# ai-forever/Kandinsky-2

Hardware: NVIDIA H100
Metric: unet_denoising_steps_per_sec (higher is better)
Workload: dtype f16

## Files before the change

kandinsky-2_b200/csrc/k2_api.cu:

```cuda
#include <stdio.h>
#include <stdlib.h>
#include <string.h>

#include <algorithm>
#include <atomic>
#include <mutex>

#include "../../include/k2b200.h"
#include "k2_internal.h"

namespace k2 {

static thread_local std::string g_err;
static std::atomic<long long> g_launches{0};
static int g_force_bn = 0;
static int g_force_split = 0;
static int g_pdl = 0;


void set_error(const std::string& msg) { g_err = msg; }
int fail(const std::string& msg) {
  g_err = msg;
  return -1;
}
// ... 316 lines not shown
                        static_cast<uint64_t>(NB)};
    uint64_t str[3] = {static_cast<uint64_t>(src.ld) * 2, static_cast<uint64_t>(src.ld) * 2 * W,
                       static_cast<uint64_t>(src.ld) * 2 * W * H};
    uint32_t box[4] = {64, static_cast<uint32_t>(p.TW), static_cast<uint32_t>(p.TH), static_cast<uint32_t>(p.TN)};
    if (encode_tmap_f16(&p.tmA[s], src.ptr, 4, dims, str, box)) return -1;
  }
  const int BN = pl.BN, splits = pl.splits, fuse_stats = pl.fuse_stats;
  p.splits = splits;
  p.k_per_split = (kchunks + splits - 1) / splits;
  p.M_total = static_cast<long long>(NB) * H * W * (up2 ? 4 : 1);
  p.ws = reinterpret_cast<float*>(workspace);
  p.n_tiles = (Cout + BN - 1) / BN;
  p.Cout = Cout;
  {
    uint64_t dims[3] = {static_cast<uint64_t>(Ktot), static_cast<uint64_t>(w_rows), static_cast<uint64_t>(w_batched ? NB : 1)};
    uint64_t str[2] = {static_cast<uint64_t>(ldw) * 2,
                       (w_batched ? static_cast<uint64_t>(w_batch_stride) : static_cast<uint64_t>(ldw) * w_rows) * 2};
    uint32_t box[3] = {64, static_cast<uint32_t>(BN), 1};
    if (encode_tmap_f16(&p.tmB, w_packed, 3, dims, str, box)) return -1;
  }
  p.bias = bias;
  p.residual = reinterpret_cast<const __half*>(residual);
  p.ldr = ldr;
  p.out = out;
  p.ldo = ldo;
  p.out_mode = (splits > 1) ? 2 : out_mode;
  p.gn_part = (fuse_stats == 1) ? reinterpret_cast<float2*>(gn_partial) : nullptr;
  p.gn_mode = (fuse_stats == 1) ? (p.TN == 1 ? 1 : 2) : 0;
  if (out_mode == 0) {
    K2_REQUIRE(ldo % 8 == 0 && (reinterpret_cast<uintptr_t>(out) & 15) == 0, "conv_gemm: out alignment");
    if (residual)
      K2_REQUIRE(ldr % 8 == 0 && (reinterpret_cast<uintptr_t>(residual) & 15) == 0, "conv_gemm: residual alignment");
  }
  int rc = launch_conv_gemm(p, BN, pl.es, static_cast<cudaStream_t>(stream));
  if (rc == 0) g_launches.fetch_add(1, std::memory_order_relaxed);
  if (rc == 0 && splits > 1) {
    rc = launch_splitk_finalize(p.ws, splits, p.M_total, Cout, bias, p.residual, ldr, reinterpret_cast<__half*>(out), ldo,
                                fuse_stats == 2 ? reinterpret_cast<float2*>(gn_partial) : nullptr,
                                static_cast<cudaStream_t>(stream));
    if (rc == 0) g_launches.fetch_add(1, std::memory_order_relaxed);
  }
  return rc;
}

int k2_conv_plan(int NB, int H, int W, int taps, int Ktot, int Cout, int out_mode, long long workspace_bytes,
                 int want_gn_partial, int* info) {
  K2_REQUIRE(NB > 0 && H > 0 && W > 0 && Cout > 0 && info, "conv_plan: bad arguments");
  K2_REQUIRE(Ktot > 0 && Ktot % 64 == 0, "conv_plan: Ktot must be a positive multiple of 64");
  ConvPlan pl;
  plan_conv(NB, H, W, taps == 9, Ktot / 64, Cout, out_mode, workspace_bytes > 0, workspace_bytes, want_gn_partial != 0, pl);
  plan_to_info(pl, info);
  return 0;
}

}
```

kandinsky-2_b200/csrc/k2_common.cuh:

```cuda
#pragma once
#include <cuda.h>
#include <cuda_fp16.h>
#include <cuda_runtime.h>
#include <stdint.h>
#include <stdio.h>

namespace k2 {

__device__ __forceinline__ uint32_t smem_u32(const void* p) {
  return static_cast<uint32_t>(__cvta_generic_to_shared(p));
}

__device__ __forceinline__ uint32_t lane_id() { return threadIdx.x & 31; }

__device__ __forceinline__ bool elect_one() {
  uint32_t pred = 0;
  asm volatile(
      "{\n"
      ".reg .b32 rx;\n"
      ".reg .pred px;\n"
      "elect.sync rx|px, 0xffffffff;\n"
      "selp.b32 %0, 1, 0, px;\n"
      "}\n"
      : "=r"(pred));
// ... 51 lines not shown
  asm volatile("fence.proxy.async.shared::cta;" ::: "memory");
}

__device__ __forceinline__ void tma_prefetch_desc(const CUtensorMap* tm) {
  asm volatile("prefetch.tensormap [%0];" ::"l"(reinterpret_cast<uint64_t>(tm)) : "memory");
}
__device__ __forceinline__ void tma_load_2d(void* dst, const CUtensorMap* tm, uint64_t* bar, int c0,
                                            int c1) {
  asm volatile(
      "cp.async.bulk.tensor.2d.shared::cluster.global.mbarrier::complete_tx::bytes [%0], [%1, {%3, "
      "%4}], [%2];"
      ::"r"(smem_u32(dst)),
      "l"(reinterpret_cast<uint64_t>(tm)), "r"(smem_u32(bar)), "r"(c0), "r"(c1)
      : "memory");
}
__device__ __forceinline__ void tma_load_3d(void* dst, const CUtensorMap* tm, uint64_t* bar, int c0,
                                            int c1, int c2) {
  asm volatile(
      "cp.async.bulk.tensor.3d.shared::cluster.global.mbarrier::complete_tx::bytes [%0], [%1, {%3, "
      "%4, %5}], [%2];"
      ::"r"(smem_u32(dst)),
      "l"(reinterpret_cast<uint64_t>(tm)), "r"(smem_u32(bar)), "r"(c0), "r"(c1), "r"(c2)
      : "memory");
}
__device__ __forceinline__ void tma_load_4d(void* dst, const CUtensorMap* tm, uint64_t* bar, int c0,
                                            int c1, int c2, int c3) {
  asm volatile(
      "cp.async.bulk.tensor.4d.shared::cluster.global.mbarrier::complete_tx::bytes [%0], [%1, {%3, "
      "%4, %5, %6}], [%2];"
      ::"r"(smem_u32(dst)),
      "l"(reinterpret_cast<uint64_t>(tm)), "r"(smem_u32(bar)), "r"(c0), "r"(c1), "r"(c2), "r"(c3)
      : "memory");
}

__device__ __forceinline__ uint64_t make_wgmma_desc(uint32_t smem_addr) {
  uint64_t d = 0;
  d |= static_cast<uint64_t>((smem_addr & 0x3FFFF) >> 4);
  d |= static_cast<uint64_t>(1) << 16;
  d |= static_cast<uint64_t>(1024 >> 4) << 32;
  d |= static_cast<uint64_t>(1) << 62;
  return d;
}
__device__ __forceinline__ void wgmma_fence() { asm volatile("wgmma.fence.sync.aligned;" ::: "memory"); }
__device__ __forceinline__ void wgmma_commit() { asm volatile("wgmma.commit_group.sync.aligned;" ::: "memory"); }
template <int N>
__device__ __forceinline__ void wgmma_wait() {
  asm volatile("wgmma.wait_group.sync.aligned %0;" ::"n"(N) : "memory");
}
__device__ __forceinline__ void wgmma_m64n16k16(float (&d)[8], uint64_t adesc, uint64_t bdesc, uint32_t accumulate) {
  asm volatile(
      "{\n"
      ".reg .pred p;\n"
      "setp.ne.b32 p, %10, 0;\n"
      "wgmma.mma_async.sync.aligned.m64n16k16.f32.f16.f16 "
      "{%0, %1, %2, %3, %4, %5, %6, %7}, %8, %9, p, 1, 1, 0, 0;\n"
      "}\n"
      : "+f"(d[0]), "+f"(d[1]), "+f"(d[2]), "+f"(d[3]), "+f"(d[4]), "+f"(d[5]), "+f"(d[6]), "+f"(d[7])
      : "l"(adesc), "l"(bdesc), "r"(accumulate));
}

__device__ __forceinline__ void wgmma_m64n64k16(float (&d)[32], uint64_t adesc, uint64_t bdesc, uint32_t accumulate) {
  asm volatile(
      "{\n"
      ".reg .pred p;\n"
      "setp.ne.b32 p, %34, 0;\n"
      "wgmma.mma_async.sync.aligned.m64n64k16.f32.f16.f16 "
// ... 99 lines not shown
  asm volatile(
      "mma.sync.aligned.m16n8k16.row.col.f32.f16.f16.f32 {%0, %1, %2, %3}, {%4, %5, %6, %7}, {%8, %9}, "
      "{%0, %1, %2, %3};"
      : "+f"(d[0]), "+f"(d[1]), "+f"(d[2]), "+f"(d[3])
      : "r"(a[0]), "r"(a[1]), "r"(a[2]), "r"(a[3]), "r"(b0), "r"(b1));
}
__device__ __forceinline__ void ldmatrix_x4(uint32_t (&r)[4], uint32_t saddr) {
  asm volatile("ldmatrix.sync.aligned.m8n8.x4.shared.b16 {%0, %1, %2, %3}, [%4];"
               : "=r"(r[0]), "=r"(r[1]), "=r"(r[2]), "=r"(r[3])
               : "r"(saddr));
}
__device__ __forceinline__ void ldmatrix_x4_trans(uint32_t (&r)[4], uint32_t saddr) {
  asm volatile("ldmatrix.sync.aligned.m8n8.x4.trans.shared.b16 {%0, %1, %2, %3}, [%4];"
               : "=r"(r[0]), "=r"(r[1]), "=r"(r[2]), "=r"(r[3])
               : "r"(saddr));
}
__device__ __forceinline__ void cp_async_16(uint32_t saddr, const void* gptr, int src_bytes) {
  asm volatile("cp.async.cg.shared.global [%0], [%1], 16, %2;" ::"r"(saddr), "l"(gptr), "r"(src_bytes) : "memory");
}
__device__ __forceinline__ void cp_async_commit() { asm volatile("cp.async.commit_group;" ::: "memory"); }
template <int N>
__device__ __forceinline__ void cp_async_wait() {
  asm volatile("cp.async.wait_group %0;" ::"n"(N) : "memory");
}

__device__ __forceinline__ void sts_v4(uint32_t saddr, uint32_t a, uint32_t b, uint32_t c, uint32_t d) {
  asm volatile("st.shared.v4.b32 [%0], {%1, %2, %3, %4};" ::"r"(saddr), "r"(a), "r"(b), "r"(c), "r"(d) : "memory");
}
__device__ __forceinline__ uint4 lds_v4(uint32_t saddr) {
  uint4 v;
  asm volatile("ld.shared.v4.b32 {%0, %1, %2, %3}, [%4];" : "=r"(v.x), "=r"(v.y), "=r"(v.z), "=r"(v.w) : "r"(saddr) : "memory");
  return v;
}
__device__ __forceinline__ uint32_t lds_u32(uint32_t saddr) {
  uint32_t v;
  asm volatile("ld.shared.b32 %0, [%1];" : "=r"(v) : "r"(saddr) : "memory");
  return v;
}
__device__ __forceinline__ void named_bar_sync(int id, int count) {
  asm volatile("bar.sync %0, %1;" ::"r"(id), "r"(count) : "memory");
}
__device__ __forceinline__ void named_bar_arrive(int id, int count) {
  asm volatile("bar.arrive %0, %1;" ::"r"(id), "r"(count) : "memory");
}
__device__ __forceinline__ void pdl_wait() { asm volatile("griddepcontrol.wait;" ::: "memory"); }
__device__ __forceinline__ void pdl_launch() { asm volatile("griddepcontrol.launch_dependents;" ::: "memory"); }

__device__ __forceinline__ float silu_f(float x) {
  float e, r;
  asm("ex2.approx.ftz.f32 %0, %1;" : "=f"(e) : "f"(-1.44269504088896341f * x));
  asm("rcp.approx.ftz.f32 %0, %1;" : "=f"(r) : "f"(1.f + e));
  return x * r;
}

}
```

kandinsky-2_b200/csrc/k2_conv_gemm.cu:

```cuda
#include <stdio.h>

#include "k2_common.cuh"
#include "k2_internal.h"

namespace k2 {

namespace {

constexpr int BM = 128;
constexpr int BK = 64;
constexpr int A_STAGE_BYTES = BM * BK * 2;
constexpr int ACC_PAD = 4;

constexpr int EPI_STAGE_FLOATS = 32 * 33;
constexpr int EPI_BYTES = 4 * EPI_STAGE_FLOATS * 4 + 4 * 256 * 4;
constexpr int SMEM_LIMIT = 227 * 1024;

template <int BN, int ES>
struct Cfg {
  static constexpr int B_STAGE_BYTES = BN * BK * 2;
  static constexpr int STAGE_BYTES = A_STAGE_BYTES + B_STAGE_BYTES;
  static constexpr int BNC = (BN < 64) ? BN : (ES == 2 ? 128 : 64);
  static_assert(ES == 1 || BN % 128 == 0, "two epilogue sets need N tiles of 128 or 256");
  static constexpr int ACC_BYTES = BM * (BNC + ACC_PAD) * 4;
  static constexpr int BAR_BYTES = 256;
  static constexpr int FIXED = ACC_BYTES + ES * EPI_BYTES + BAR_BYTES + 1024;
  static constexpr int STAGES = (SMEM_LIMIT - FIXED) / STAGE_BYTES > 6 ? 6 : (SMEM_LIMIT - FIXED) / STAGE_BYTES;
  static constexpr int SMEM_BYTES = STAGES * STAGE_BYTES + FIXED;
  static_assert(STAGES >= 2, "conv_gemm: shared memory does not hold two pipeline stages");
};

__device__ __forceinline__ void decode_m_tile(const ConvGemmParams& p, int m_idx, int& n0, int& y0,
                                              int& x0, int& phase) {
  phase = 0;
  if (p.up2) {
    phase = m_idx / p.m_tiles_phase;
    m_idx -= phase * p.m_tiles_phase;
  }
  int tw_i = m_idx % p.tiles_w;
  int t = m_idx / p.tiles_w;
  int th_i = t % p.tiles_h;
  int tn_i = t / p.tiles_h;
  x0 = tw_i * p.TW;
  y0 = th_i * p.TH;
  n0 = tn_i * p.TN;
}

template <int N>
__device__ __forceinline__ void acc_ld(const float* src, uint32_t (&r)[N]) {
#pragma unroll
  for (int v = 0; v < N / 4; ++v) {
    const float4 t = *reinterpret_cast<const float4*>(src + 4 * v);
    r[4 * v] = __float_as_uint(t.x);
    r[4 * v + 1] = __float_as_uint(t.y);
    r[4 * v + 2] = __float_as_uint(t.z);
    r[4 * v + 3] = __float_as_uint(t.w);
  }
}

template <int BN, int ES>
// ... 243 lines not shown
                }
                uint4 ov;
                __half2* oh = reinterpret_cast<__half2*>(&ov);
#pragma unroll
                for (int e = 0; e < 4; ++e) oh[e] = __floats2half2_rn(f[2 * e], f[2 * e + 1]);
                *reinterpret_cast<uint4*>(orow + v * 8) = ov;
              }
            } else {
#pragma unroll
              for (int e = 0; e < CH; ++e) {
                if (col0 + e < p.Cout) {
                  float f = __uint_as_float(r[e]);
                  if (p.bias) f += __ldg(p.bias + col0 + e);
                  if (rrow) f += __half2float(rrow[e]);
                  orow[e] = __float2half_rn(f);
                }
              }
            }
          } else {
            float* o = reinterpret_cast<float*>(p.out);
#pragma unroll
            for (int e = 0; e < CH; ++e) {
              if (col0 + e < p.Cout) {
                float f = __uint_as_float(r[e]);
                if (p.bias) f += __ldg(p.bias + col0 + e);
                o[((static_cast<long long>(n) * p.Cout + (col0 + e)) * p.H + y) * p.W + x] = f;
              }
            }
          }
        }
      }
}


template <int BN, int ES>
__global__ void __launch_bounds__(384, 1) conv_gemm_kernel(const __grid_constant__ ConvGemmParams p) {
  using C = Cfg<BN, ES>;
  constexpr int BNC = C::BNC;
  constexpr int NA = BN / 2;
  extern __shared__ uint8_t smem_raw[];
  uint8_t* smem = reinterpret_cast<uint8_t*>((reinterpret_cast<uintptr_t>(smem_raw) + 1023) &
                                             ~static_cast<uintptr_t>(1023));
  float* acc_smem = reinterpret_cast<float*>(smem + C::STAGES * C::STAGE_BYTES);
  float* stat_smem = reinterpret_cast<float*>(smem + C::STAGES * C::STAGE_BYTES + C::ACC_BYTES);
  uint64_t* full_bar = reinterpret_cast<uint64_t*>(smem + C::STAGES * C::STAGE_BYTES + C::ACC_BYTES + ES * EPI_BYTES);
  uint64_t* empty_bar = full_bar + C::STAGES;

  const int warp_idx = threadIdx.x >> 5;
  const int lane = threadIdx.x & 31;
  const int wg = warp_idx >> 2;

  if (threadIdx.x == 0) {
    tma_prefetch_desc(&p.tmB);
    for (int s = 0; s < 3; ++s)
      if (p.seg_taps[s]) tma_prefetch_desc(&p.tmA[s]);
    for (int i = 0; i < C::STAGES; ++i) {
      mbar_init(&full_bar[i], 1);
      mbar_init(&empty_bar[i], 8);
    }
    fence_barrier_init();
  }
  __syncthreads();
  pdl_wait();
  pdl_launch();

  const int total_tiles = p.m_tiles * p.n_tiles * p.splits;

  if (wg == 0) {
    setmaxnreg_dec<40>();
    if (warp_idx == 0 && elect_one()) {
      int stage = 0;
      uint32_t ring_phase = 0;
      const uint32_t tx_bytes = p.a_box_bytes + C::B_STAGE_BYTES;
      for (int tile = blockIdx.x; tile < total_tiles; tile += gridDim.x) {
        const int n_idx = tile % p.n_tiles;
        const int m_idx = (tile / p.n_tiles) % p.m_tiles;
        const int split = tile / (p.m_tiles * p.n_tiles);
        int n0, y0, x0, phase;
        decode_m_tile(p, m_idx, n0, y0, x0, phase);
        const int kb = phase * p.num_k_chunks;
        const int k0 = split * p.k_per_split;
        const int k1 = min(p.num_k_chunks, k0 + p.k_per_split);
        int s = 0, rem = k0;
        while (rem >= p.seg_taps[s] * p.seg_kchunks[s]) {
          rem -= p.seg_taps[s] * p.seg_kchunks[s];
          ++s;
        }
        int tap = rem / p.seg_kchunks[s];
        int c = rem - tap * p.seg_kchunks[s];
        for (int kc = k0; kc < k1; ++kc) {
          const int taps = p.seg_taps[s];
          const int dy = (taps == 9) ? (tap / 3 - 1) : (taps == 4 ? (tap >> 1) + (phase >> 1) - 1 : 0);
          const int dx = (taps == 9) ? (tap % 3 - 1) : (taps == 4 ? (tap & 1) + (phase & 1) - 1 : 0);
          mbar_wait_lean(&empty_bar[stage], ring_phase ^ 1);
          uint8_t* sA = smem + stage * C::STAGE_BYTES;
          uint8_t* sB = sA + A_STAGE_BYTES;
          mbar_arrive_expect_tx(&full_bar[stage], tx_bytes);
          tma_load_4d(sA, &p.tmA[s], &full_bar[stage], c * BK, x0 + dx, y0 + dy, n0);
          tma_load_3d(sB, &p.tmB, &full_bar[stage], (kb + kc) * BK, n_idx * BN, p.w_batched ? n0 : 0);
          if (++stage == C::STAGES) {
            stage = 0;
            ring_phase ^= 1;
          }
          if (++c == p.seg_kchunks[s]) {
            c = 0;
            if (++tap == taps) {
              tap = 0;
              ++s;
            }
          }
        }
      }
    }
  } else {
    setmaxnreg_inc<232>();
    const int g = wg - 1;
    const int w = warp_idx & 3;
    int stage = 0;
    uint32_t phase = 0;
    for (int tile = blockIdx.x; tile < total_tiles; tile += gridDim.x) {
      const int n_idx = tile % p.n_tiles;
      const int m_idx = (tile / p.n_tiles) % p.m_tiles;
      const int split = tile / (p.m_tiles * p.n_tiles);
      const int nk = min(p.num_k_chunks, (split + 1) * p.k_per_split) - split * p.k_per_split;
      float acc[NA];
#pragma unroll
      for (int i = 0; i < NA; ++i) acc[i] = 0.f;
      int prev_stage = -1;
      for (int kc = 0; kc < nk; ++kc) {
        mbar_wait_lean(&full_bar[stage], phase);
        const uint32_t a_addr = smem_u32(smem + stage * C::STAGE_BYTES) + g * (64 * 128);
        const uint32_t b_addr = smem_u32(smem + stage * C::STAGE_BYTES + A_STAGE_BYTES);
        wgmma_fence();
#pragma unroll
        for (int k = 0; k < BK / 16; ++k) {
          const uint64_t adesc = make_wgmma_desc(a_addr) + static_cast<uint64_t>(k * 2);
          const uint64_t bdesc = make_wgmma_desc(b_addr) + static_cast<uint64_t>(k * 2);
          if constexpr (BN == 256) {
            wgmma_m64n256k16(acc, adesc, bdesc, 1u);
          } else if constexpr (BN == 192) {
            wgmma_m64n192k16(acc, adesc, bdesc, 1u);
          } else if constexpr (BN == 128) {
            wgmma_m64n128k16(acc, adesc, bdesc, 1u);
          } else if constexpr (BN == 64) {
            wgmma_m64n64k16(acc, adesc, bdesc, 1u);
          } else {
            static_assert(BN == 16, "conv_gemm: N tile without a wgmma shape");
            wgmma_m64n16k16(acc, adesc, bdesc, 1u);
          }
        }
        wgmma_commit();
        wgmma_wait<1>();
        if (prev_stage >= 0 && lane == 0) mbar_arrive(&empty_bar[prev_stage]);
        prev_stage = stage;
        if (++stage == C::STAGES) {
          stage = 0;
          phase ^= 1;
        }
      }
      wgmma_wait<0>();
      if (prev_stage >= 0 && lane == 0) mbar_arrive(&empty_bar[prev_stage]);

      int n0, y0, x0, mphase;
      decode_m_tile(p, m_idx, n0, y0, x0, mphase);
      const int r0 = 64 * g + 16 * w + (lane >> 2);
      const int cq = 2 * (lane & 3);
#pragma unroll
      for (int pass = 0; pass < BN / BNC; ++pass) {
        named_bar_sync(3, 256);
#pragma unroll
        for (int i = 0; i < NA; i += 2) {
          if ((8 * (i >> 2)) / BNC != pass) continue;
          const int row = r0 + 8 * ((i >> 1) & 1);
          const int col = 8 * (i >> 2) - pass * BNC + cq;
          *reinterpret_cast<float2*>(acc_smem + row * (BNC + ACC_PAD) + col) = make_float2(acc[i], acc[i + 1]);
        }
        named_bar_sync(3, 256);
        if (ES == 2 || g == 0)
          epilogue_tile<BNC, ES>(p, acc_smem, w, lane, n0, y0, x0, n_idx * BN + pass * BNC, split, m_idx, stat_smem, g,
                                 mphase);
      }
    }
  }
}

__global__ void __launch_bounds__(256) splitk_finalize_kernel(const float* __restrict__ ws, int splits, long long M,
                                                              int Cout, const float* __restrict__ bias,
                                                              const __half* __restrict__ residual, int ldr,
                                                              __half* __restrict__ out, int ldo, float2* __restrict__ gn_part) {
  __shared__ float red[8][32][17];
  const int vx = threadIdx.x & 31, ry = threadIdx.x >> 5;
  const int c0 = (blockIdx.y * 32 + vx) * 8;
  const long long rg = blockIdx.x;
  pdl_wait();
  pdl_launch();
  float st[16];
#pragma unroll
  for (int e = 0; e < 16; ++e) st[e] = 0.f;
  if (c0 < Cout) {
    float bv[8];
#pragma unroll
    for (int e = 0; e < 8; ++e) bv[e] = bias ? __ldg(bias + c0 + e) : 0.f;
#pragma unroll
    for (int rr = 0; rr < 2; ++rr) {
      const long long m = rg * 16 + ry + rr * 8;
      if (m >= M) continue;
      float f[8];
#pragma unroll
      for (int e = 0; e < 8; ++e) f[e] = bv[e];
      for (int s = 0; s < splits; ++s) {
        const float4* w = reinterpret_cast<const float4*>(ws + (static_cast<long long>(s) * M + m) * Cout + c0);
        const float4 a = __ldcs(w), b = __ldcs(w + 1);
        f[0] += a.x; f[1] += a.y; f[2] += a.z; f[3] += a.w; f[4] += b.x; f[5] += b.y; f[6] += b.z; f[7] += b.w;
// ... 10 lines not shown
      }
      uint4 ov;
      __half2* oh = reinterpret_cast<__half2*>(&ov);
#pragma unroll
      for (int e = 0; e < 4; ++e) {
        oh[e] = __floats2half2_rn(f[2 * e], f[2 * e + 1]);
        const float2 t = __half22float2(oh[e]);
        st[2 * e] += t.x;
        st[2 * e + 1] += t.y;
        st[8 + 2 * e] = fmaf(t.x, t.x, st[8 + 2 * e]);
        st[8 + 2 * e + 1] = fmaf(t.y, t.y, st[8 + 2 * e + 1]);
      }
      *reinterpret_cast<uint4*>(out + m * ldo + c0) = ov;
    }
  }
  if (gn_part == nullptr) return;
#pragma unroll
  for (int e = 0; e < 16; ++e) red[ry][vx][e] = st[e];
  __syncthreads();
  const int vx2 = threadIdx.x >> 3, e2 = threadIdx.x & 7;
  const int c = (blockIdx.y * 32 + vx2) * 8 + e2;
  if (c < Cout) {
    float s1 = 0.f, s2 = 0.f;
#pragma unroll
    for (int q = 0; q < 8; ++q) {
      s1 += red[q][vx2][e2];
      s2 += red[q][vx2][8 + e2];
    }
    gn_part[rg * Cout + c] = make_float2(s1, s2);
  }
}


template <int BN, int ES>
int launch_bn(const ConvGemmParams& p, cudaStream_t stream) {
  using C = Cfg<BN, ES>;
  static bool attr_set = false;
  if (!attr_set) {
    K2_CHECK_CUDA(cudaFuncSetAttribute(conv_gemm_kernel<BN, ES>, cudaFuncAttributeMaxDynamicSharedMemorySize,
                                       C::SMEM_BYTES));
    attr_set = true;
  }
  int total = p.m_tiles * p.n_tiles * p.splits;
  int grid = total < num_sms() ? total : num_sms();
  K2_CHECK_CUDA(launch_k(conv_gemm_kernel<BN, ES>, dim3(grid), dim3(384), C::SMEM_BYTES, stream, p));
  return 0;
}

}

int launch_splitk_finalize(const float* ws, int splits, long long M, int Cout, const float* bias, const __half* residual,
                           int ldr, __half* out, int ldo, float2* gn_part, cudaStream_t stream) {
  dim3 grid(static_cast<unsigned int>((M + 15) / 16), (Cout / 8 + 31) / 32);
  K2_CHECK_CUDA(launch_k(splitk_finalize_kernel, grid, dim3(256), 0, stream, ws, splits, M, Cout, bias, residual, ldr, out, ldo,
                         gn_part));
  return 0;
}

int launch_conv_gemm(const ConvGemmParams& p, int BN, int epilogue_sets, cudaStream_t stream) {
  if (epilogue_sets == 2) {
    switch (BN) {
      case 128: return launch_bn<128, 2>(p, stream);
      case 256: return launch_bn<256, 2>(p, stream);
      default: break;
    }
  }
  switch (BN) {
    case 16: return launch_bn<16, 1>(p, stream);
    case 64: return launch_bn<64, 1>(p, stream);
    case 128: return launch_bn<128, 1>(p, stream);
    case 192: return launch_bn<192, 1>(p, stream);
    case 256: return launch_bn<256, 1>(p, stream);
    default: return fail("conv_gemm: unsupported BN");
  }
}

}
```

kandinsky-2_b200/csrc/k2_internal.h:

```cpp
#pragma once
#include <cuda.h>
#include <cuda_fp16.h>
#include <cuda_runtime.h>
#include <stdint.h>

#include <string>

namespace k2 {

void set_error(const std::string& msg);
int fail(const std::string& msg);
#define K2_CHECK_CUDA(expr)                                                                 \
  do {                                                                                      \
    cudaError_t _e = (expr);                                                                \
    if (_e != cudaSuccess)                                                                  \
      return ::k2::fail(std::string(#expr) + ": " + cudaGetErrorString(_e));                \
  } while (0)
#define K2_REQUIRE(cond, msg)                                  \
  do {                                                         \
    if (!(cond)) return ::k2::fail(std::string("k2b200: ") + (msg)); \
  } while (0)

inline bool aligned16(const void* p) { return (reinterpret_cast<uintptr_t>(p) & 15) == 0; }

// ... 17 lines not shown
}
void count_launch(int n = 1);

int encode_tmap_f16(CUtensorMap* out, const void* base, int rank, const uint64_t* dims,
                    const uint64_t* strides_bytes , const uint32_t* box);

struct ConvGemmParams {
  CUtensorMap tmA[3];
  CUtensorMap tmB;
  int w_batched;
  int seg_taps[3];
  int seg_kchunks[3];
  int num_k_chunks;
  int NB, H, W;
  int TN, TH, TW;
  int tiles_n, tiles_h, tiles_w;
  int m_tiles, n_tiles;
  int Cout;
  const float* bias;
  const __half* residual;
  int ldr;
  void* out;
  int ldo;
  int out_mode;
  uint32_t a_box_bytes;
  int splits;
  int k_per_split;
  float* ws;
  long long M_total;
  float2* gn_part;
  int gn_mode;
  int up2;
  int m_tiles_phase;
};
int launch_conv_gemm(const ConvGemmParams& p, int BN, int epilogue_sets, cudaStream_t stream);
int launch_splitk_finalize(const float* ws, int splits, long long M, int Cout, const float* bias, const __half* residual,
                           int ldr, __half* out, int ldo, float2* gn_part, cudaStream_t stream);

struct FlashParams {
  const __half* qkv;
  long long ldq;
  int hs, q_off, k_off, v_off;
  const __half* enc;
  long long lde;
  int ehs, ek_off, ev_off;
  int B, heads, T, Tc;
  __half* out;
  int ldo, ohs;
  float scale_log2e;
};
int gn_apply_blocks_per_sm();
int launch_attention(const FlashParams& p, int head_dim, cudaStream_t stream);

}
```

kandinsky-2_b200/kandinsky2/launch_plan.py:

```python
import gc
import os

import torch

from . import ops

FOLD_MAX_RG = int(os.environ.get("K2_GN_FOLD_MAX_RG", "18"))
TUNE = os.environ.get("K2_AUTOTUNE", "1") != "0"
FORK = os.environ.get("K2_FORK", "1") != "0"
TUNE_SMALL_M = int(os.environ.get("K2_TUNE_SMALL_M", "8192"))
_tune_cache = {}


def tune(key, run, m_rows=0):
    if not TUNE:
        return None
    key = (torch.cuda.current_device(), TUNE_SMALL_M) + key
    if key in _tune_cache:
        return _tune_cache[key]
    info = [0] * 7
    run(None, info)
    bn0, splits = info[0], info[2]
    cout = key[3]
    best = None
    if cout > 64:
        bns = [bn0] if splits > 1 else [bn for bn in (128, 192, 256) if bn - 64 < cout or bn == bn0]
        cands = [(bn0, 0, splits, 1)] + [(bn, 0, splits, es) for bn in bns for es in ((1,) if bn == 192 else (1, 2))
                                        if (bn, es) != (bn0, 1)]
        if 0 < m_rows <= TUNE_SMALL_M and splits == 1:
            for bn in (128, 192, 256):
                if bn - 64 >= cout:
                    continue
                for sp in (2, 3, 4):
                    probe = [0] * 7
                    try:
                        run((bn, 1, sp, 1), probe)
                    except Exception:
                        continue
                    if probe[0] == bn and probe[2] == sp:
                        cands.append((bn, 1, sp, 1))

        def timed(cfg, reps=6):
            run(cfg)
            evs = [torch.cuda.Event(enable_timing=True) for _ in range(reps + 1)]
            evs[0].record()
            for i in range(reps):
                run(cfg)
                evs[i + 1].record()
            torch.cuda.synchronize()
            return min(evs[i].elapsed_time(evs[i + 1]) for i in range(reps))

        t0 = tb = timed(cands[0])
        for cfg in cands[1:]:
            t = timed(cfg)
            if t < tb and t < 0.97 * t0:
                t = max(t, timed(cfg))
                if t < tb and t < 0.97 * t0:
                    best, tb = cfg, t
    _tune_cache[key] = best
    return best
# ... 39 lines not shown
                ev = torch.cuda.Event()
                ev.record()
                self._side_stream.wait_event(ev)
            with torch.cuda.stream(self._side_stream):
                fn()
        self._add(step, kind, flops)

    def _join(self):
        if not self._side_open:
            return
        self._side_open = False

        def step():
            if self._serial:
                return
            ev = torch.cuda.Event()
            ev.record(self._side_stream)
            torch.cuda.current_stream().wait_event(ev)
        self._add(step, "join", 0)

    def _conv(self, srcs, w, cout, out, flops, bias=None, residual=None, want_stats=True, part_slot=None, out_mode=0,
              geom=None, w_batch_stride=0, kind="conv_gemm"):
        part = None
        if want_stats and out_mode == 0:
            g = geom if geom is not None else tuple(out.shape[:3])
            n = ops.gn_part_floats(g[0], g[1], g[2], cout)
            part = self._tmp(part_slot, n, dtype=torch.float32) if part_slot else self._new(n, dtype=torch.float32)
        info = [0] * 7
        run = lambda cfg, info=None: ops.conv_gemm(srcs, w, cout, bias=bias, residual=residual, out=out, gn_part=part,
                                                   info=info, cfg=cfg, out_mode=out_mode, geom=geom,
                                                   w_batch_stride=w_batch_stride)
        key = ("conv", cout, tuple(out.shape), geom, tuple((t.shape[-1], taps) for t, taps in srcs), residual is not None,
               part is not None, out_mode, w_batch_stride > 0)
        cfg = tune(key, run, m_rows=out.shape[0] * out.shape[1] * out.shape[2] if out_mode == 0 and geom is None else 0)
        self._add(lambda: run(cfg, info), kind, flops)
        if part is not None and info[5]:
            self._parts[out.data_ptr()] = (part, info[6] // (geom[0] if geom is not None else out.shape[0]))
        else:
            self._parts.pop(out.data_ptr(), None)

    def _gemm(self, x, w, cout, out, flops, bias=None, residual=None):
        run = lambda cfg, info=None: ops.gemm_rows(x, w, cout, bias=bias, residual=residual, out=out, cfg=cfg, info=info)
        cfg = tune(("gemm", cout, tuple(x.shape), residual is not None), run, m_rows=x.shape[0] * x.shape[1])
        self._add(lambda: run(cfg), "conv_gemm", flops)
        self._parts.pop(out.data_ptr(), None)

    def _stats(self, a, b, eps):
        pa = self._parts.get(a.data_ptr())
        pb = self._parts.get(b.data_ptr()) if b is not None else None
        st = self._new(self.NB, 32, 2, dtype=torch.float32)
        HW = a.shape[1] * a.shape[2]
        if pa is not None and (b is None or pb is not None):
            c1 = b.shape[-1] if b is not None else 0
            self._add(lambda: ops.gn_finalize(pa[0], a.shape[-1], pb[0] if pb else None, c1, self.NB, pa[1], HW, st,
                                              rg1=pb[1] if pb else None, eps=eps), "gn_finalize")
        else:
            self._add(lambda: ops.gn_stats(a, b, stats=st, eps=eps), "gn_stats")
        return st

    def _norm(self, a, b, gamma, beta, y, film=None, act=1, resample=0, xres=None, eps=1e-5):
        pa = self._parts.get(a.data_ptr())
        pb = self._parts.get(b.data_ptr()) if b is not None else None
        have = pa is not None and (b is None or pb is not None)
        cpg = (a.shape[-1] + (b.shape[-1] if b is not None else 0)) // 32
        if have and cpg >= 2 and max(pa[1], pb[1] if pb else 0) <= FOLD_MAX_RG:
            self._add(lambda: ops.gn_apply_fold(a, b, pa[0], pa[1], pb[0] if pb else None, pb[1] if pb else 0, gamma, beta,
                                                film=film, act=act, resample=resample, y=y, xres=xres, eps=eps), "gn_apply")
# ... 66 lines not shown
```

profiles/conv_layers.py:

```python
import argparse
import json
import os
import subprocess
import sys

ROOT = os.path.dirname(os.path.dirname(os.path.abspath(__file__)))
for p in (ROOT, os.path.join(ROOT, "kandinsky-2_b200")):
    if p not in sys.path:
        sys.path.insert(0, p)

import torch

B, H, W = 4, 96, 96


def _card():
    q = subprocess.run(["nvidia-smi", "--query-gpu=name,power.limit,clocks.max.sm", "--format=csv,noheader", "-i", "0"],
                       capture_output=True, text=True)
    return q.stdout.strip() or torch.cuda.get_device_name(0)


def _pad64(c):
    return (c + 63) // 64 * 64

# ... 48 lines not shown
        run(cfg)
    e.record()
    torch.cuda.synchronize()
    reps = max(10, int(min_ms / max(s.elapsed_time(e) / 5, 1e-3)) + 1)
    s.record()
    for _ in range(reps):
        run(cfg)
    e.record()
    torch.cuda.synchronize()
    return s.elapsed_time(e) / reps, reps


def main():
    ap = argparse.ArgumentParser()
    ap.add_argument("--out", default=None)
    ap.add_argument("--min-ms", type=float, default=50.0, help="timed window per configuration")
    ap.add_argument("--mma-n", default="tile", choices=["tile", "64"],
                    help="wgmma N of the build: one instruction per N tile, or m64n64k16 per 64 columns")
    args = ap.parse_args()
    if not torch.cuda.is_available():
        raise SystemExit("needs a CUDA sm_90 device")
    import bench
    from kandinsky2 import launch_plan, ops
    from kandinsky2.model.gaussian_diffusion import FusedStep, create_ddpm_v22
    dev = torch.device("cuda", 0)
    torch.cuda.set_device(dev)
    ops.set_tuning(4, 1)
    res = {"card": _card(), "torch": torch.__version__, "geometry": f"cfg-2: UNet batch {2 * B}, {H}x{W} latents",
           "mma_n": args.mma_n, "min_ms": args.min_ms}

    counts = {}
    tune = launch_plan.tune

    def counting_tune(key, run, m_rows=0):
        counts[key] = counts.get(key, 0) + 1
        return tune(key, run, m_rows=m_rows)
    launch_plan.tune = counting_tune
    model = bench.build_unet(dev)
    image_emb = torch.randn(2 * B, 1280, generator=torch.Generator().manual_seed(1234)).to(dev)
    step = FusedStep(model, B, H, W, dict(image_emb=image_emb), guidance_scale=4.0, cond_first=False, clip_range=2.0,
                     threshold_mode=0)
    launch_plan.tune = tune
    diffusion = create_ddpm_v22(50)
    coef, ts = diffusion._tables(dev)
    order = torch.arange(diffusion.num_timesteps - 1, -1, -1, device=dev)
    step.set_schedule(ts[order], coef[order], torch.randn(len(order), B, 4, H, W, device=dev))
    x = step.latent()
    x.copy_(torch.randn(B, 4, H, W, device=dev))
    step.advance(x)
    torch.cuda.synchronize()
    res["plan_conv_launches"] = sum(1 for _, kind, _ in step.plan.steps if kind == "conv_gemm")
    res["counted_conv_launches"] = sum(counts.values())

    g = torch.Generator(device=dev).manual_seed(7)
    layers = []
    for key, n in counts.items():
        run, shp = _layer(key, dev, g)
        if run is None:
            continue
        info = [0] * 7
        picked = launch_plan._tune_cache.get((dev.index, launch_plan.TUNE_SMALL_M) + key)
        run(picked, info)
        picked_cfg = [info[0], 0, info[2], (picked[3] if picked and picked[3] else 1)]
        cout = shp["N"]
        cfgs = []
        if cout > 64:
            cfgs = [(bn, 0, 1, es) for bn in (128, 192, 256) if bn - 64 < cout or bn == info[0]
                    for es in ((1,) if bn == 192 else (1, 2))]
        if tuple(picked_cfg) not in cfgs:
# ... 49 lines not shown
```

Before: 31.14.

## Add TMA-store epilogue for conv GEMM with TMA-loaded residual and smem GN stats

Adds a new epilogue path for non-split, non-upsampled direct-output convolutions. The consumer warpgroups convert accumulators to fp16 and add bias and a residual that was prefetched by TMA into a swizzled shared-memory D tile. Producer-group warps then issue TMA tensor stores and compute the GroupNorm partials from that tile. This drops the fp32 accumulator staging buffer and the per-thread global stores, and the next tile's residual load overlaps with the current tile's work. It also moves the PDL launch_dependents trigger to the last tile and stops tuning two epilogue sets for plain convolutions. The cost is higher register pressure, changed setmaxnreg splits, and a serialization point on the single D tile between tiles.

```diff
diff --git a/kandinsky-2_b200/csrc/k2_api.cu b/kandinsky-2_b200/csrc/k2_api.cu
--- a/kandinsky-2_b200/csrc/k2_api.cu
+++ b/kandinsky-2_b200/csrc/k2_api.cu
@@ -372,6 +372,19 @@
     if (residual)
       K2_REQUIRE(ldr % 8 == 0 && (reinterpret_cast<uintptr_t>(residual) & 15) == 0, "conv_gemm: residual alignment");
   }
+  if (conv_tma_epilogue(p, BN)) {
+    uint64_t dims[4] = {static_cast<uint64_t>(Cout), static_cast<uint64_t>(W), static_cast<uint64_t>(H),
+                        static_cast<uint64_t>(NB)};
+    uint32_t box[4] = {64, static_cast<uint32_t>(p.TW), static_cast<uint32_t>(p.TH), static_cast<uint32_t>(p.TN)};
+    uint64_t str[3] = {static_cast<uint64_t>(ldo) * 2, static_cast<uint64_t>(ldo) * 2 * W,
+                       static_cast<uint64_t>(ldo) * 2 * W * H};
+    if (encode_tmap_f16(&p.tmOut, out, 4, dims, str, box)) return -1;
+    if (residual) {
+      uint64_t rstr[3] = {static_cast<uint64_t>(ldr) * 2, static_cast<uint64_t>(ldr) * 2 * W,
+                          static_cast<uint64_t>(ldr) * 2 * W * H};
+      if (encode_tmap_f16(&p.tmRes, residual, 4, dims, rstr, box)) return -1;
+    }
+  }
   int rc = launch_conv_gemm(p, BN, pl.es, static_cast<cudaStream_t>(stream));
   if (rc == 0) g_launches.fetch_add(1, std::memory_order_relaxed);
   if (rc == 0 && splits > 1) {
diff --git a/kandinsky-2_b200/csrc/k2_common.cuh b/kandinsky-2_b200/csrc/k2_common.cuh
--- a/kandinsky-2_b200/csrc/k2_common.cuh
+++ b/kandinsky-2_b200/csrc/k2_common.cuh
@@ -107,6 +107,15 @@
       "l"(reinterpret_cast<uint64_t>(tm)), "r"(smem_u32(bar)), "r"(c0), "r"(c1), "r"(c2), "r"(c3)
       : "memory");
 }
+
+__device__ __forceinline__ void tma_store_4d(const void* src, const CUtensorMap* tm, int c0, int c1, int c2, int c3) {
+  asm volatile("cp.async.bulk.tensor.4d.global.shared::cta.bulk_group [%0, {%2, %3, %4, %5}], [%1];"
+               ::"l"(reinterpret_cast<uint64_t>(tm)), "r"(smem_u32(src)), "r"(c0), "r"(c1), "r"(c2), "r"(c3)
+               : "memory");
+}
+__device__ __forceinline__ void bulk_commit() { asm volatile("cp.async.bulk.commit_group;" ::: "memory"); }
+__device__ __forceinline__ void bulk_wait_read_all() { asm volatile("cp.async.bulk.wait_group.read 0;" ::: "memory"); }
+__device__ __forceinline__ void bulk_wait_all() { asm volatile("cp.async.bulk.wait_group 0;" ::: "memory"); }
 
 __device__ __forceinline__ uint64_t make_wgmma_desc(uint32_t smem_addr) {
   uint64_t d = 0;
@@ -272,6 +281,9 @@
   asm volatile("ld.shared.v4.b32 {%0, %1, %2, %3}, [%4];" : "=r"(v.x), "=r"(v.y), "=r"(v.z), "=r"(v.w) : "r"(saddr) : "memory");
   return v;
 }
+__device__ __forceinline__ void sts_u32(uint32_t saddr, uint32_t v) {
+  asm volatile("st.shared.b32 [%0], %1;" ::"r"(saddr), "r"(v) : "memory");
+}
 __device__ __forceinline__ uint32_t lds_u32(uint32_t saddr) {
   uint32_t v;
   asm volatile("ld.shared.b32 %0, [%1];" : "=r"(v) : "r"(saddr) : "memory");
diff --git a/kandinsky-2_b200/csrc/k2_conv_gemm.cu b/kandinsky-2_b200/csrc/k2_conv_gemm.cu
--- a/kandinsky-2_b200/csrc/k2_conv_gemm.cu
+++ b/kandinsky-2_b200/csrc/k2_conv_gemm.cu
@@ -16,16 +16,20 @@
 constexpr int EPI_BYTES = 4 * EPI_STAGE_FLOATS * 4 + 4 * 256 * 4;
 constexpr int SMEM_LIMIT = 227 * 1024;
 
-template <int BN, int ES>
+template <int BN, int ES, bool TE>
 struct Cfg {
   static constexpr int B_STAGE_BYTES = BN * BK * 2;
   static constexpr int STAGE_BYTES = A_STAGE_BYTES + B_STAGE_BYTES;
   static constexpr int BNC = (BN < 64) ? BN : (ES == 2 ? 128 : 64);
   static_assert(ES == 1 || BN % 128 == 0, "two epilogue sets need N tiles of 128 or 256");
-  static constexpr int ACC_BYTES = BM * (BNC + ACC_PAD) * 4;
+  static_assert(!TE || (ES == 1 && BN % 64 == 0), "the TMA epilogue stores 64-column boxes");
+  static constexpr int ACC_BYTES = TE ? 0 : BM * (BNC + ACC_PAD) * 4;
+  static constexpr int EPI_SMEM = TE ? 0 : ES * EPI_BYTES;
+  static constexpr int D_BYTES = TE ? BM * BN * 2 : 0;
   static constexpr int BAR_BYTES = 256;
-  static constexpr int FIXED = ACC_BYTES + ES * EPI_BYTES + BAR_BYTES + 1024;
-  static constexpr int STAGES = (SMEM_LIMIT - FIXED) / STAGE_BYTES > 6 ? 6 : (SMEM_LIMIT - FIXED) / STAGE_BYTES;
+  static constexpr int FIXED = ACC_BYTES + EPI_SMEM + D_BYTES + BAR_BYTES + 1024;
+  static constexpr int STAGE_MAX = TE ? Cfg<BN, 1, false>::STAGES : 6;
+  static constexpr int STAGES = (SMEM_LIMIT - FIXED) / STAGE_BYTES > STAGE_MAX ? STAGE_MAX : (SMEM_LIMIT - FIXED) / STAGE_BYTES;
   static constexpr int SMEM_BYTES = STAGES * STAGE_BYTES + FIXED;
   static_assert(STAGES >= 2, "conv_gemm: shared memory does not hold two pipeline stages");
 };
@@ -335,10 +339,72 @@
       }
 }
 
-
-template <int BN, int ES>
+__device__ __forceinline__ uint32_t dtile_off(int row, int col) {
+  return (col >> 6) * (BM * 128) + row * 128 + ((((col >> 3) & 7) ^ (row & 7)) << 4) + (col & 7) * 2;
+}
+
+template <int BN>
+__device__ __forceinline__ void dtile_prepare(const ConvGemmParams& p, int tile, uint8_t* dtile, uint64_t* d_ready) {
+  if (!p.residual) {
+    mbar_arrive(d_ready);
+    return;
+  }
+  const int n_idx = tile % p.n_tiles;
+  const int m_idx = (tile / p.n_tiles) % p.m_tiles;
+  int n0, y0, x0, phase;
+  decode_m_tile(p, m_idx, n0, y0, x0, phase);
+  const int c0 = n_idx * BN;
+  const int nbox = min(BN / 64, (p.Cout - c0 + 63) / 64);
+  mbar_arrive_expect_tx(d_ready, nbox * p.a_box_bytes);
+  for (int j = 0; j < nbox; ++j) tma_load_4d(dtile + j * (BM * 128), &p.tmRes, d_ready, c0 + 64 * j, x0, y0, n0);
+}
+
+template <int BN>
+__device__ __forceinline__ void dtile_gn_partials(const ConvGemmParams& p, uint32_t dtile, int kw, int lane, int n_idx,
+                                                  int m_idx, int n0) {
+#pragma unroll 1
+  for (int jp = kw; jp < BN / 64; jp += 3) {
+    const int col0 = n_idx * BN + jp * 64;
+    if (col0 >= p.Cout) break;
+    float4 fold = make_float4(0.f, 0.f, 0.f, 0.f);
+#pragma unroll 1
+    for (int ew = 0; ew < 4; ++ew) {
+      float4 h0 = make_float4(0.f, 0.f, 0.f, 0.f), h1 = make_float4(0.f, 0.f, 0.f, 0.f);
+#pragma unroll
+      for (int rr = 0; rr < 32; ++rr) {
+        const uint32_t w = lds_u32(dtile + dtile_off(ew * 32 + rr, jp * 64 + 2 * lane));
+        const float2 t = __half22float2(*reinterpret_cast<const __half2*>(&w));
+        float4& hacc = (rr < 16) ? h0 : h1;
+        hacc.x += t.x;
+        hacc.y = fmaf(t.x, t.x, hacc.y);
+        hacc.z += t.y;
+        hacc.w = fmaf(t.y, t.y, hacc.w);
+      }
+      if (p.gn_mode == 2) {
+        const int per = p.tiles_h * p.tiles_w;
+        const int sp = m_idx % per;
+        const int img = n0 + 2 * ew;
+        if (2 * ew < p.TN && img < p.NB)
+          *reinterpret_cast<float4*>(p.gn_part + (static_cast<long long>(img) * per + sp) * p.Cout + col0 + 2 * lane) = h0;
+        if (2 * ew + 1 < p.TN && img + 1 < p.NB)
+          *reinterpret_cast<float4*>(p.gn_part + (static_cast<long long>(img + 1) * per + sp) * p.Cout + col0 + 2 * lane) = h1;
+      } else {
+        const float4 t = make_float4(h0.x + h1.x, h0.y + h1.y, h0.z + h1.z, h0.w + h1.w);
+        fold.x += t.x; fold.y += t.y; fold.z += t.z; fold.w += t.w;
+      }
+    }
+    if (p.gn_mode == 1)
+      *reinterpret_cast<float4*>(p.gn_part + static_cast<long long>(m_idx) * p.Cout + col0 + 2 * lane) = fold;
+  }
+}
+
+constexpr int BAR_D_WRITTEN = 4;
+constexpr int BAR_D_READ = 5;
+
+
+template <int BN, int ES, bool TE>
 __global__ void __launch_bounds__(384, 1) conv_gemm_kernel(const __grid_constant__ ConvGemmParams p) {
-  using C = Cfg<BN, ES>;
+  using C = Cfg<BN, ES, TE>;
   constexpr int BNC = C::BNC;
   constexpr int NA = BN / 2;
   extern __shared__ uint8_t smem_raw[];
@@ -346,8 +412,11 @@
                                              ~static_cast<uintptr_t>(1023));
   float* acc_smem = reinterpret_cast<float*>(smem + C::STAGES * C::STAGE_BYTES);
   float* stat_smem = reinterpret_cast<float*>(smem + C::STAGES * C::STAGE_BYTES + C::ACC_BYTES);
-  uint64_t* full_bar = reinterpret_cast<uint64_t*>(smem + C::STAGES * C::STAGE_BYTES + C::ACC_BYTES + ES * EPI_BYTES);
+  uint8_t* dtile = smem + C::STAGES * C::STAGE_BYTES;
+  uint64_t* full_bar =
+      reinterpret_cast<uint64_t*>(smem + C::STAGES * C::STAGE_BYTES + C::ACC_BYTES + C::EPI_SMEM + C::D_BYTES);
   uint64_t* empty_bar = full_bar + C::STAGES;
+  uint64_t* d_ready = empty_bar + C::STAGES;
 
   const int warp_idx = threadIdx.x >> 5;
   const int lane = threadIdx.x & 31;
@@ -361,16 +430,20 @@
       mbar_init(&full_bar[i], 1);
       mbar_init(&empty_bar[i], 8);
     }
+    if constexpr (TE) {
+      tma_prefetch_desc(&p.tmOut);
+      if (p.residual) tma_prefetch_desc(&p.tmRes);
+      mbar_init(d_ready, 1);
+    }
     fence_barrier_init();
   }
   __syncthreads();
   pdl_wait();
-  pdl_launch();
 
   const int total_tiles = p.m_tiles * p.n_tiles * p.splits;
 
   if (wg == 0) {
-    setmaxnreg_dec<40>();
+    if constexpr (TE) setmaxnreg_dec<56>(); else setmaxnreg_dec<40>();
     if (warp_idx == 0 && elect_one()) {
       int stage = 0;
       uint32_t ring_phase = 0;
@@ -414,13 +487,40 @@
           }
         }
       }
+    } else if (TE && warp_idx > 0) {
+      const bool issuer = warp_idx == 1 && lane == 0;
+      const uint32_t dt = smem_u32(dtile);
+      if (issuer && static_cast<int>(blockIdx.x) < total_tiles) dtile_prepare<BN>(p, blockIdx.x, dtile, d_ready);
+      for (int tile = blockIdx.x; tile < total_tiles; tile += gridDim.x) {
+        const int n_idx = tile % p.n_tiles;
+        const int m_idx = (tile / p.n_tiles) % p.m_tiles;
+        int n0, y0, x0, phase;
+        decode_m_tile(p, m_idx, n0, y0, x0, phase);
+        named_bar_sync(BAR_D_WRITTEN, 352);
+        if (issuer) {
+          const int c0 = n_idx * BN;
+          const int nbox = min(BN / 64, (p.Cout - c0 + 63) / 64);
+          for (int j = 0; j < nbox; ++j) tma_store_4d(dtile + j * (BM * 128), &p.tmOut, c0 + 64 * j, x0, y0, n0);
+          bulk_commit();
+        }
+        if (p.gn_part) {
+          dtile_gn_partials<BN>(p, dt, warp_idx - 1, lane, n_idx, m_idx, n0);
+          named_bar_sync(BAR_D_READ, 96);
+        }
+        if (issuer) {
+          bulk_wait_read_all();
+          if (tile + static_cast<int>(gridDim.x) < total_tiles) dtile_prepare<BN>(p, tile + gridDim.x, dtile, d_ready);
+        }
+      }
+      if (issuer) bulk_wait_all();
     }
   } else {
-    setmaxnreg_inc<232>();
+    if constexpr (TE) setmaxnreg_inc<224>(); else setmaxnreg_inc<232>();
     const int g = wg - 1;
     const int w = warp_idx & 3;
     int stage = 0;
     uint32_t phase = 0;
+    uint32_t tile_parity = 0;
     for (int tile = blockIdx.x; tile < total_tiles; tile += gridDim.x) {
       const int n_idx = tile % p.n_tiles;
       const int m_idx = (tile / p.n_tiles) % p.m_tiles;
@@ -463,25 +563,77 @@
       }
       wgmma_wait<0>();
       if (prev_stage >= 0 && lane == 0) mbar_arrive(&empty_bar[prev_stage]);
+      if (tile + static_cast<int>(gridDim.x) >= total_tiles) pdl_launch();
 
       int n0, y0, x0, mphase;
       decode_m_tile(p, m_idx, n0, y0, x0, mphase);
       const int r0 = 64 * g + 16 * w + (lane >> 2);
       const int cq = 2 * (lane & 3);
-#pragma unroll
-      for (int pass = 0; pass < BN / BNC; ++pass) {
-        named_bar_sync(3, 256);
-#pragma unroll
-        for (int i = 0; i < NA; i += 2) {
-          if ((8 * (i >> 2)) / BNC != pass) continue;
-          const int row = r0 + 8 * ((i >> 1) & 1);
-          const int col = 8 * (i >> 2) - pass * BNC + cq;
-          *reinterpret_cast<float2*>(acc_smem + row * (BNC + ACC_PAD) + col) = make_float2(acc[i], acc[i + 1]);
-        }
-        named_bar_sync(3, 256);
-        if (ES == 2 || g == 0)
-          epilogue_tile<BNC, ES>(p, acc_smem, w, lane, n0, y0, x0, n_idx * BN + pass * BNC, split, m_idx, stat_smem, g,
-                                 mphase);
+      if constexpr (TE) {
+#pragma unroll
+        for (int i = 0; i < NA; ++i) reg_fence(acc[i]);
+        bool valid[2];
+#pragma unroll
+        for (int h = 0; h < 2; ++h) {
+          const int row = r0 + 8 * h;
+          const int thw = p.TH * p.TW;
+          const int tn = row / thw, th = (row - tn * thw) / p.TW, tw = row - tn * thw - th * p.TW;
+          valid[h] = (tn < p.TN) && (n0 + tn < p.NB) && (y0 + th < p.H) && (x0 + tw < p.W);
+        }
+        const uint32_t dt = smem_u32(dtile);
+        const int cbase = n_idx * BN;
+        mbar_wait_lean(d_ready, tile_parity);
+        tile_parity ^= 1;
+#pragma unroll
+        for (int jb = 0; jb < BN / 64; ++jb) {
+          uint32_t v[16];
+#pragma unroll
+          for (int k = 0; k < 16; ++k) {
+            const int i = 32 * jb + 2 * k;
+            v[k] = p.residual ? lds_u32(dt + dtile_off(r0 + 8 * ((i >> 1) & 1), 8 * (i >> 2) + cq)) : 0u;
+          }
+#pragma unroll
+          for (int k = 0; k < 16; ++k) {
+            const int i = 32 * jb + 2 * k;
+            const int h = (i >> 1) & 1;
+            const int col = 8 * (i >> 2) + cq;
+            float f0 = acc[i], f1 = acc[i + 1];
+            if (p.bias) {
+              if (cbase + col < p.Cout) f0 += __ldg(p.bias + cbase + col);
+              if (cbase + col + 1 < p.Cout) f1 += __ldg(p.bias + cbase + col + 1);
+            }
+            if (p.residual) {
+              const float2 t = __half22float2(*reinterpret_cast<const __half2*>(&v[k]));
+              f0 += t.x;
+              f1 += t.y;
+            }
+            const __half2 hh = __floats2half2_rn(f0, f1);
+            v[k] = valid[h] ? *reinterpret_cast<const uint32_t*>(&hh) : 0u;
+          }
+#pragma unroll
+          for (int k = 0; k < 16; ++k) {
+            const int i = 32 * jb + 2 * k;
+            sts_u32(dt + dtile_off(r0 + 8 * ((i >> 1) & 1), 8 * (i >> 2) + cq), v[k]);
+          }
+        }
+        fence_proxy_async_smem();
+        named_bar_arrive(BAR_D_WRITTEN, 352);
+      } else {
+#pragma unroll
+        for (int pass = 0; pass < BN / BNC; ++pass) {
+          named_bar_sync(3, 256);
+#pragma unroll
+          for (int i = 0; i < NA; i += 2) {
+            if ((8 * (i >> 2)) / BNC != pass) continue;
+            const int row = r0 + 8 * ((i >> 1) & 1);
+            const int col = 8 * (i >> 2) - pass * BNC + cq;
+            *reinterpret_cast<float2*>(acc_smem + row * (BNC + ACC_PAD) + col) = make_float2(acc[i], acc[i + 1]);
+          }
+          named_bar_sync(3, 256);
+          if (ES == 2 || g == 0)
+            epilogue_tile<BNC, ES>(p, acc_smem, w, lane, n0, y0, x0, n_idx * BN + pass * BNC, split, m_idx, stat_smem, g,
+                                   mphase);
+        }
       }
     }
   }
@@ -558,18 +710,23 @@
 }
 
 
-template <int BN, int ES>
+template <int BN, int ES, bool TE = false>
 int launch_bn(const ConvGemmParams& p, cudaStream_t stream) {
-  using C = Cfg<BN, ES>;
+  using C = Cfg<BN, ES, TE>;
   static bool attr_set = false;
   if (!attr_set) {
-    K2_CHECK_CUDA(cudaFuncSetAttribute(conv_gemm_kernel<BN, ES>, cudaFuncAttributeMaxDynamicSharedMemorySize,
+    K2_CHECK_CUDA(cudaFuncSetAttribute(conv_gemm_kernel<BN, ES, TE>, cudaFuncAttributeMaxDynamicSharedMemorySize,
                                        C::SMEM_BYTES));
     attr_set = true;
   }
   int total = p.m_tiles * p.n_tiles * p.splits;
   int grid = total < num_sms() ? total : num_sms();
-  K2_CHECK_CUDA(launch_k(conv_gemm_kernel<BN, ES>, dim3(grid), dim3(384), C::SMEM_BYTES, stream, p));
+  cudaLaunchConfig_t cfg = {};
+  cfg.gridDim = dim3(grid);
+  cfg.blockDim = dim3(384);
+  cfg.dynamicSmemBytes = C::SMEM_BYTES;
+  cfg.stream = stream;
+  K2_CHECK_CUDA(cudaLaunchKernelEx(&cfg, conv_gemm_kernel<BN, ES, TE>, p));
   return 0;
 }
 
@@ -584,6 +741,15 @@
 }
 
 int launch_conv_gemm(const ConvGemmParams& p, int BN, int epilogue_sets, cudaStream_t stream) {
+  if (conv_tma_epilogue(p, BN)) {
+    switch (BN) {
+      case 64: return launch_bn<64, 1, true>(p, stream);
+      case 128: return launch_bn<128, 1, true>(p, stream);
+      case 192: return launch_bn<192, 1, true>(p, stream);
+      case 256: return launch_bn<256, 1, true>(p, stream);
+      default: return fail("conv_gemm: unsupported BN");
+    }
+  }
   if (epilogue_sets == 2) {
     switch (BN) {
       case 128: return launch_bn<128, 2>(p, stream);
diff --git a/kandinsky-2_b200/csrc/k2_internal.h b/kandinsky-2_b200/csrc/k2_internal.h
--- a/kandinsky-2_b200/csrc/k2_internal.h
+++ b/kandinsky-2_b200/csrc/k2_internal.h
@@ -73,7 +73,12 @@
   int gn_mode;
   int up2;
   int m_tiles_phase;
+  CUtensorMap tmOut;
+  CUtensorMap tmRes;
 };
+inline bool conv_tma_epilogue(const ConvGemmParams& p, int BN) {
+  return p.out_mode == 0 && p.splits == 1 && !p.up2 && BN >= 64;
+}
 int launch_conv_gemm(const ConvGemmParams& p, int BN, int epilogue_sets, cudaStream_t stream);
 int launch_splitk_finalize(const float* ws, int splits, long long M, int Cout, const float* bias, const __half* residual,
                            int ldr, __half* out, int ldo, float2* gn_part, cudaStream_t stream);
diff --git a/kandinsky-2_b200/kandinsky2/launch_plan.py b/kandinsky-2_b200/kandinsky2/launch_plan.py
--- a/kandinsky-2_b200/kandinsky2/launch_plan.py
+++ b/kandinsky-2_b200/kandinsky2/launch_plan.py
@@ -12,7 +12,7 @@
 _tune_cache = {}
 
 
-def tune(key, run, m_rows=0):
+def tune(key, run, m_rows=0, staged=False):
     if not TUNE:
         return None
     key = (torch.cuda.current_device(), TUNE_SMALL_M) + key
@@ -25,7 +25,8 @@
     best = None
     if cout > 64:
         bns = [bn0] if splits > 1 else [bn for bn in (128, 192, 256) if bn - 64 < cout or bn == bn0]
-        cands = [(bn0, 0, splits, 1)] + [(bn, 0, splits, es) for bn in bns for es in ((1,) if bn == 192 else (1, 2))
+        sets = (1, 2) if staged or splits > 1 else (1,)
+        cands = [(bn0, 0, splits, 1)] + [(bn, 0, splits, es) for bn in bns for es in ((1,) if bn == 192 else sets)
                                         if (bn, es) != (bn0, 1)]
         if 0 < m_rows <= TUNE_SMALL_M and splits == 1:
             for bn in (128, 192, 256):
@@ -131,7 +132,8 @@
                                                    w_batch_stride=w_batch_stride)
         key = ("conv", cout, tuple(out.shape), geom, tuple((t.shape[-1], taps) for t, taps in srcs), residual is not None,
                part is not None, out_mode, w_batch_stride > 0)
-        cfg = tune(key, run, m_rows=out.shape[0] * out.shape[1] * out.shape[2] if out_mode == 0 and geom is None else 0)
+        cfg = tune(key, run, m_rows=out.shape[0] * out.shape[1] * out.shape[2] if out_mode == 0 and geom is None else 0,
+                   staged=out_mode != 0 or srcs[0][1] == 4)
         self._add(lambda: run(cfg, info), kind, flops)
         if part is not None and info[5]:
             self._parts[out.data_ptr()] = (part, info[6] // (geom[0] if geom is not None else out.shape[0]))
diff --git a/profiles/conv_layers.py b/profiles/conv_layers.py
--- a/profiles/conv_layers.py
+++ b/profiles/conv_layers.py
@@ -104,9 +104,9 @@
     counts = {}
     tune = launch_plan.tune
 
-    def counting_tune(key, run, m_rows=0):
+    def counting_tune(key, run, m_rows=0, **kw):
         counts[key] = counts.get(key, 0) + 1
-        return tune(key, run, m_rows=m_rows)
+        return tune(key, run, m_rows=m_rows, **kw)
     launch_plan.tune = counting_tune
     model = bench.build_unet(dev)
     image_emb = torch.randn(2 * B, 1280, generator=torch.Generator().manual_seed(1234)).to(dev)
```

Measured after the change: 32.35, median of 6. 1.04x the previous value.
